# savelovme/adaptive-mcmc

Measured on AMD Instinct MI355X. Metric: chain-steps/sec (whole node) + ESS/sec, 64-dim Gaussian, higher is better.
Workload: dtype f32; 1 GPU; ARWMH.sample, d=64 correlated Gaussian, 65536 chains, per-chain adaptation (BASELINE.json configs[1]); chains_per_gpu=65536, dim=64, parallelism=1 GPU

## Files before the change

adaptive-mcmc_amd/csrc/amh_step64.hip:

```cpp
#include "amh_asss.h"
#include "amh_device.h"
#include "amh_s64_sched.h"
#include "amh_step_stage.h"

namespace amh {

#ifdef AMH_STAMPS
constexpr int kS64StampWaves = 1 << 16;
constexpr int kS64StampSlots = 8;
__device__ unsigned long long g_s64_stamps[kS64StampWaves * kS64StampSlots];
hipError_t diag_s64_stamps_copy(void* host, size_t bytes) {
  return hipMemcpyFromSymbol(host, HIP_SYMBOL(g_s64_stamps), bytes, 0, hipMemcpyDeviceToHost);
}
#define AMH_S64_PHASE_INIT unsigned long long st_ph[4] = {0, 0, 0, 0}, st_pt = 0;
#define AMH_S64_PHASE_MARK st_pt = __builtin_amdgcn_s_memrealtime();
#define AMH_S64_PHASE(k)                                             \
  {                                                                  \
    const unsigned long long t_ = __builtin_amdgcn_s_memrealtime();  \
    st_ph[k] += t_ - st_pt;                                          \
    st_pt = t_;                                                      \
  }
#else
#define AMH_S64_PHASE_INIT
#define AMH_S64_PHASE_MARK
#define AMH_S64_PHASE(k)
#endif

constexpr int kS64Waves = 16;
constexpr int kS64LoadAuxHot = 2, kS64LoadAuxCold = 2;
constexpr int kS64StoreAuxHot = 2, kS64StoreAuxMid = 0, kS64StoreAuxTail = 0;
constexpr int kS64TagShift = 60;
constexpr int64_t kS64IdxMask = ((int64_t)1 << kS64TagShift) - 1;
__device__ __forceinline__ int s64_cls(int64_t t) { return (int)(t >> kS64TagShift); }
template <class F>
__device__ __forceinline__ void s64_load_policy(int cls, F&& f) {
  using std::integral_constant;
  if constexpr (kS64LoadAuxHot == kS64LoadAuxCold) {
    f(integral_constant<int, kS64LoadAuxCold>{});
  } else {
    if (cls & (int)kS64Hot) f(integral_constant<int, kS64LoadAuxHot>{});
    else f(integral_constant<int, kS64LoadAuxCold>{});
  }
}
template <class F>
__device__ __forceinline__ void s64_store_policy(int cls, F&& f) {
  using std::integral_constant;
  if constexpr (kS64StoreAuxHot == kS64StoreAuxMid && kS64StoreAuxTail == kS64StoreAuxMid) {
    f(integral_constant<int, kS64StoreAuxMid>{});
  } else {
    if (cls & (int)kS64Hot) f(integral_constant<int, kS64StoreAuxHot>{});
    else if (cls & (int)kS64Tail) f(integral_constant<int, kS64StoreAuxTail>{});
    else f(integral_constant<int, kS64StoreAuxMid>{});
  }
}
constexpr int kS64EB = 8;
constexpr int kS64PB = 8;
static_assert(kS64EB == 8 && kS64PB == 8, "the batch readers (lds_ld4x2w / lds_ld4x4w) read two quarter-vectors per stream");
typedef uint32_t uint32x4_t_ __attribute__((ext_vector_type(4)));
constexpr int kS64P = 2080;
constexpr int kS64Z = 2080, kS64M = 2144, kS64S = 2208, kS64X = 2216;
constexpr int kS64WB = kS64X + 64;
constexpr int kS64Model = 64 * 68;
static_assert(kS64Z == 2080 && kS64S == kS64M + 64, "layout of prefetch_item<64>");
template <int WPB = kS64Waves>
constexpr size_t s64_lds_bytes() { return ((size_t)kS64Model + (size_t)WPB * kS64WB + 32) * sizeof(float); }

constexpr int s64_col(int j) { return j * 64 - j * (j - 1) / 2; }

constexpr int kS64Pieces = 9;
constexpr int s64_piece_end(int m) { return m < kS64Pieces - 1 ? 256 * (m + 1) : kS64P; }
constexpr int s64_piece_group(int m) {
  for (int g = 0; g < 16; ++g)
    if (s64_col(4 * g + 4) >= s64_piece_end(m)) return g;
  return -1;
}
constexpr int s64_piece_after(int g) {
  for (int m = 0; m < kS64Pieces; ++m)
    if (s64_piece_group(m) == g) return m;
  return -1;
}
constexpr bool s64_pieces_ok() {
  int n = 0;
  for (int g = 0; g < 16; ++g) n += s64_piece_after(g) >= 0;
  for (int m = 0; m + 1 < kS64Pieces; ++m)
    if (s64_piece_group(m) < 0 || s64_piece_group(m) >= s64_piece_group(m + 1)) return false;
  return n == kS64Pieces;
}
static_assert(256 * (kS64Pieces - 1) <= kS64P && kS64P - 256 * (kS64Pieces - 1) <= 64, "eight 1-KB pieces and a one-DMA tail");
static_assert(s64_col(64) == kS64P && s64_pieces_ok(), "every piece is finished by its own swap group, in order");
static_assert(s64_piece_group(0) == 1 && s64_piece_group(4) == 6 && s64_piece_group(7) == 14 &&
                  s64_piece_group(kS64Pieces - 1) == 15,
              "the table of DESIGN.md 3.1");

#define AMH_SWG_RD(k) "s_lshl_b64 exec, -1, %[m" #k "]\n\tds_read_b32 %[t" #k "], %[la] offset:%[o" #k "]\n\t"
#define AMH_SWG_RD_HEAD "ds_read_b128 %[dl], %[zm] offset:%[od]\n\tds_read_b128 %[in], %[zm] offset:%[oi]\n\t"
#define AMH_SWG_RD_PIECE "ds_read_b128 %[pv], %[lp] offset:%[op]\n\t"
#define AMH_SWG_RD_TAIL "s_mov_b64 exec, -1\n\ts_waitcnt lgkmcnt(0)"
template <int G, int MP>
__device__ __forceinline__ void s64_group_read(f32x4& dl4, f32x4& in4, f32x4& pv, float (&t)[4], uint32_t zm_a,
                                               uint32_t la16, uint32_t la) {
  constexpr int j = 4 * G;
  static_assert(G < 15 || MP >= 0, "the last group reads the piece that group 14 finished");
#define AMH_SWG_RD_OPS3                                                                                       \
  [zm] "v"(zm_a), [la] "v"(la), [od] "n"(16 * G), [oi] "n"(256 + 16 * G), [m0] "n"(j + 1), [m1] "n"(j + 2), \
      [m2] "n"(j + 3), [o0] "n"((s64_col(j) - j) * 4), [o1] "n"((s64_col(j + 1) - (j + 1)) * 4),             \
      [o2] "n"((s64_col(j + 2) - (j + 2)) * 4)
  if constexpr (G == 15) {
    asm volatile(AMH_SWG_RD_HEAD AMH_SWG_RD_PIECE AMH_SWG_RD(0) AMH_SWG_RD(1) AMH_SWG_RD(2) AMH_SWG_RD_TAIL
                 : [dl] "=&v"(dl4), [in] "=&v"(in4), [pv] "=&v"(pv), [t0] "=&v"(t[0]), [t1] "=&v"(t[1]),
                   [t2] "=&v"(t[2])
                 : AMH_SWG_RD_OPS3, [lp] "v"(la16), [op] "n"(1024 * MP));
  } else if constexpr (MP >= 0) {
    asm volatile(AMH_SWG_RD_HEAD AMH_SWG_RD_PIECE AMH_SWG_RD(0) AMH_SWG_RD(1) AMH_SWG_RD(2) AMH_SWG_RD(3)
                     AMH_SWG_RD_TAIL
                 : [dl] "=&v"(dl4), [in] "=&v"(in4), [pv] "=&v"(pv), [t0] "=&v"(t[0]), [t1] "=&v"(t[1]),
                   [t2] "=&v"(t[2]), [t3] "=&v"(t[3])
                 : AMH_SWG_RD_OPS3, [m3] "n"(j + 4), [o3] "n"((s64_col(j + 3) - (j + 3)) * 4), [lp] "v"(la16),
                   [op] "n"(1024 * MP));
  } else {
    asm volatile(AMH_SWG_RD_HEAD AMH_SWG_RD(0) AMH_SWG_RD(1) AMH_SWG_RD(2) AMH_SWG_RD(3) AMH_SWG_RD_TAIL
                 : [dl] "=&v"(dl4), [in] "=&v"(in4), [t0] "=&v"(t[0]), [t1] "=&v"(t[1]), [t2] "=&v"(t[2]),
                   [t3] "=&v"(t[3])
                 : AMH_SWG_RD_OPS3, [m3] "n"(j + 4), [o3] "n"((s64_col(j + 3) - (j + 3)) * 4));
  }
#undef AMH_SWG_RD_OPS3
}
#define AMH_SWG_LP                                                                      \
  "v_mul_f32 %[d0], %[u0], %[d0]\n\tv_mul_f32 %[d1], %[u1], %[d1]\n\t"                  \
  "v_mul_f32 %[d2], %[u2], %[d2]\n\tv_mul_f32 %[d3], %[u3], %[d3]\n\t"
#define AMH_SWG_WR(k) "ds_write_b32 %[la], %[d" #k "] offset:%[o" #k "]\n\t"
#define AMH_SWG_NRM(k) "v_mul_f32 %[u" #k "], %[t" #k "], %[i" #k "]\n\t"
#define AMH_SWG_SH(k) "s_lshl_b64 exec, -1, %[m" #k "]\n\t"
#define AMH_SWG_OFFS                                                                                          \
  [o0] "n"((s64_col(j) - j) * 4), [o1] "n"((s64_col(j + 1) - (j + 1)) * 4),                                   \
      [o2] "n"((s64_col(j + 2) - (j + 2)) * 4), [o3] "n"((s64_col(j + 3) - (j + 3)) * 4), [m0] "n"(j),        \
      [m1] "n"(j + 1), [m2] "n"(j + 2), [m3] "n"(j + 3)
template <int G>
__device__ __forceinline__ void s64_group_write(const float (&U)[64], uint32_t la, const f32x4& dl4) {
  constexpr int j = 4 * G;
  float d0 = dl4[0], d1 = dl4[1], d2 = dl4[2], d3 = dl4[3];
  asm volatile(AMH_SWG_LP AMH_SWG_SH(0) AMH_SWG_WR(0) AMH_SWG_SH(1) AMH_SWG_WR(1) AMH_SWG_SH(2) AMH_SWG_WR(2)
                   AMH_SWG_SH(3) AMH_SWG_WR(3) "s_mov_b64 exec, -1"
               : [d0] "+v"(d0), [d1] "+v"(d1), [d2] "+v"(d2), [d3] "+v"(d3)
               : [la] "v"(la), [u0] "v"(U[j]), [u1] "v"(U[j + 1]), [u2] "v"(U[j + 2]), [u3] "v"(U[j + 3]), AMH_SWG_OFFS
               : "memory");
}
template <int G>
__device__ __forceinline__ void s64_group_norm(float (&U)[64], const f32x4& in4, const float (&t)[4]) {
  constexpr int j = 4 * G;
  if constexpr (G < 15) {
    asm volatile(AMH_SWG_SH(1) AMH_SWG_NRM(0) AMH_SWG_SH(2) AMH_SWG_NRM(1) AMH_SWG_SH(3) AMH_SWG_NRM(2) AMH_SWG_SH(4)
                     AMH_SWG_NRM(3) "s_mov_b64 exec, -1"
                 : [u0] "+v"(U[j]), [u1] "+v"(U[j + 1]), [u2] "+v"(U[j + 2]), [u3] "+v"(U[j + 3])
                 : [t0] "v"(t[0]), [t1] "v"(t[1]), [t2] "v"(t[2]), [t3] "v"(t[3]), [i0] "v"(in4[0]), [i1] "v"(in4[1]),
                   [i2] "v"(in4[2]), [i3] "v"(in4[3]), [m1] "n"(j + 1), [m2] "n"(j + 2), [m3] "n"(j + 3),
                   [m4] "n"(j + 4));
  } else {
    asm volatile(AMH_SWG_SH(1) AMH_SWG_NRM(0) AMH_SWG_SH(2) AMH_SWG_NRM(1) AMH_SWG_SH(3) AMH_SWG_NRM(2)
                 "s_mov_b64 exec, -1"
                 : [u0] "+v"(U[j]), [u1] "+v"(U[j + 1]), [u2] "+v"(U[j + 2])
                 : [t0] "v"(t[0]), [t1] "v"(t[1]), [t2] "v"(t[2]), [i0] "v"(in4[0]), [i1] "v"(in4[1]),
                   [i2] "v"(in4[2]), [m1] "n"(j + 1), [m2] "n"(j + 2), [m3] "n"(j + 3));
  }
}
template <int O0, int O1>
__device__ __forceinline__ void lds_ld4x2w(f32x4& a, f32x4& b, uint32_t addr) {
  asm volatile("ds_read_b128 %0, %2 offset:%3\n\tds_read_b128 %1, %2 offset:%4\n\ts_waitcnt lgkmcnt(0)"
               : "=&v"(a), "=&v"(b)
               : "v"(addr), "n"(O0), "n"(O1));
}
template <int O0, int O1, int O2, int O3>
__device__ __forceinline__ void lds_ld4x4w(f32x4& a, f32x4& b, f32x4& c, f32x4& d, uint32_t addr0, uint32_t addr1) {
  asm volatile("ds_read_b128 %0, %4 offset:%6\n\tds_read_b128 %1, %4 offset:%7\n\t"
               "ds_read_b128 %2, %5 offset:%8\n\tds_read_b128 %3, %5 offset:%9\n\ts_waitcnt lgkmcnt(0)"
               : "=&v"(a), "=&v"(b), "=&v"(c), "=&v"(d)
               : "v"(addr0), "v"(addr1), "n"(O0), "n"(O1), "n"(O2), "n"(O3));
}

#define AMH_SW1_COL(k)                                                          \
  "s_lshl_b64 exec, -1, %[s" #k "]\n\tv_readlane_b32 %[t], %[w], %[l" #k "]\n\t" \
  "s_nop 1\n\tv_fma_f32 %[w], -%[t], %[u" #k "], %[w]\n\ts_nop 0\n\t"
template <int J0>
__device__ __forceinline__ void s64_sweep1x8(float& w, const float (&U)[64]) {
  uint64_t sv;
  uint32_t t;
  if constexpr (J0 + 7 <= 62) {
    asm volatile("s_mov_b64 %[sv], exec\n\t" AMH_SW1_COL(0) AMH_SW1_COL(1) AMH_SW1_COL(2) AMH_SW1_COL(3)
                 AMH_SW1_COL(4) AMH_SW1_COL(5) AMH_SW1_COL(6) AMH_SW1_COL(7) "s_mov_b64 exec, %[sv]"
                 : [w] "+v"(w), [t] "=&s"(t), [sv] "=&s"(sv)
                 : [u0] "v"(U[J0]), [u1] "v"(U[J0 + 1]), [u2] "v"(U[J0 + 2]), [u3] "v"(U[J0 + 3]),
                   [u4] "v"(U[J0 + 4]), [u5] "v"(U[J0 + 5]), [u6] "v"(U[J0 + 6]), [u7] "v"(U[J0 + 7]),
                   [s0] "n"(J0 + 1), [s1] "n"(J0 + 2), [s2] "n"(J0 + 3), [s3] "n"(J0 + 4), [s4] "n"(J0 + 5),
                   [s5] "n"(J0 + 6), [s6] "n"(J0 + 7), [s7] "n"(J0 + 8), [l0] "n"(J0), [l1] "n"(J0 + 1),
                   [l2] "n"(J0 + 2), [l3] "n"(J0 + 3), [l4] "n"(J0 + 4), [l5] "n"(J0 + 5), [l6] "n"(J0 + 6),
                   [l7] "n"(J0 + 7));
  } else {
    static_assert(J0 == 56, "sweep 1 covers columns 0 .. 62");
    asm volatile("s_mov_b64 %[sv], exec\n\t" AMH_SW1_COL(0) AMH_SW1_COL(1) AMH_SW1_COL(2) AMH_SW1_COL(3)
                 AMH_SW1_COL(4) AMH_SW1_COL(5) AMH_SW1_COL(6) "s_mov_b64 exec, %[sv]"
                 : [w] "+v"(w), [t] "=&s"(t), [sv] "=&s"(sv)
                 : [u0] "v"(U[J0]), [u1] "v"(U[J0 + 1]), [u2] "v"(U[J0 + 2]), [u3] "v"(U[J0 + 3]),
                   [u4] "v"(U[J0 + 4]), [u5] "v"(U[J0 + 5]), [u6] "v"(U[J0 + 6]), [s0] "n"(J0 + 1),
                   [s1] "n"(J0 + 2), [s2] "n"(J0 + 3), [s3] "n"(J0 + 4), [s4] "n"(J0 + 5), [s5] "n"(J0 + 6),
                   [s6] "n"(J0 + 7), [l0] "n"(J0), [l1] "n"(J0 + 1), [l2] "n"(J0 + 2), [l3] "n"(J0 + 3),
                   [l4] "n"(J0 + 4), [l5] "n"(J0 + 5), [l6] "n"(J0 + 6));
  }
}
#undef AMH_SW1_COL
__device__ __forceinline__ void s64_sweep1_all(float& w, const float (&U)[64]) {
  static_for<8>([&](auto B) {
    s64_sweep1x8<8 * B>(w, U);
    __builtin_amdgcn_sched_barrier(0);
  });
}

template <int Q>
__device__ __forceinline__ void s64_wr4_quarter(uint32_t a, float v0, float v1, float v2, float v3) {
  uint64_t sv;
  asm volatile("s_mov_b64 %0, exec\n\ts_bfm_b64 exec, 16, %6\n\tds_write_b32 %1, %2\n\t"
               "ds_write_b32 %1, %3 offset:64\n\tds_write_b32 %1, %4 offset:128\n\t"
               "ds_write_b32 %1, %5 offset:192\n\ts_mov_b64 exec, %0"
               : "=&s"(sv) : "v"(a), "v"(v0), "v"(v1), "v"(v2), "v"(v3), "n"(16 * Q) : "memory");
}
__device__ __forceinline__ void s64_wr(uint32_t a, float v) {
  asm volatile("ds_write_b32 %0, %1" : : "v"(a), "v"(v) : "memory");
}
template <int OFF>
__device__ __forceinline__ void s64_wr_off(uint32_t a, float v) {
  asm volatile("ds_write_b32 %0, %1 offset:%2" : : "v"(a), "v"(v), "n"(OFF) : "memory");
}
__device__ __forceinline__ void s64_wait() { asm volatile("s_waitcnt lgkmcnt(0)" ::: "memory"); }
template <class T>
__device__ __forceinline__ void s64_tie(T& a) { asm volatile("s_waitcnt lgkmcnt(0)" : "+v"(a)); }
template <class T>
__device__ __forceinline__ void s64_tie(T& a, T& b) { asm volatile("s_waitcnt lgkmcnt(0)" : "+v"(a), "+v"(b)); }

template <int J>
__device__ __forceinline__ float s64_keep_at(float old, float v) {
  float out;
  unsigned long long m;
  asm("s_lshl_b64 %1, 1, %4\n\tv_cndmask_b32_e64 %0, %2, %3, %1" : "=v"(out), "=&s"(m) : "v"(old), "v"(v), "n"(J));
  return out;
}

template <bool WAIT = false>
__device__ __forceinline__ float s64_matvec(const float (&U)[64], float h, uint32_t x_a, uint32_t r) {
  s64_wr(x_a + r * 4u, h);
  float a4[4] = {0.0f, 0.0f, 0.0f, 0.0f};
  static_for<64 / kS64EB>([&](auto B) {
    constexpr int b = B;
    f32x4 e[kS64EB / 4];
    lds_ld4x2w<16 * (2 * b), 16 * (2 * b + 1)>(e[0], e[1], x_a);
    static_for<kS64EB>([&](auto K) {
      constexpr int j = kS64EB * b + K;
      a4[j & 3] = fmaf(U[j], e[(int)K / 4][(int)K % 4], a4[j & 3]);
    });
    __builtin_amdgcn_sched_barrier(0);
  });
  if constexpr (WAIT) s64_wait();
  return (a4[0] + a4[1]) + (a4[2] + a4[3]);
}

__device__ __forceinline__ float s64_gauss_pot(float diff, uint32_t x_a, uint32_t prow, uint32_t r, float c0) {
  s64_wr(x_a + r * 4u, diff);
  f32x2v y01 = {0.0f, 0.0f}, y23 = {0.0f, 0.0f};
  static_for<64 / kS64PB>([&](auto B) {
    constexpr int b = B;
    constexpr int NQ = kS64PB / 4;
    f32x4 pv[NQ], dv[NQ];
    lds_ld4x4w<16 * (2 * b), 16 * (2 * b + 1), 16 * (2 * b), 16 * (2 * b + 1)>(pv[0], pv[1], dv[0], dv[1], prow, x_a);
    static_for<2 * NQ>([&](auto K2) {
      const f32x4 q = pv[(int)K2 / 2];
      const f32x4 dq = dv[(int)K2 / 2];
      const f32x2v pp = (K2 % 2 == 0) ? f32x2v{q[0], q[1]} : f32x2v{q[2], q[3]};
      const f32x2v bp = (K2 % 2 == 0) ? f32x2v{dq[0], dq[1]} : f32x2v{dq[2], dq[3]};
      if constexpr (K2 % 2 == 0) {
        y01 = __builtin_elementwise_fma(pp, bp, y01);
      } else {
        y23 = __builtin_elementwise_fma(pp, bp, y23);
      }
    });
    __builtin_amdgcn_sched_barrier(0);
  });
  const float y = (y01[0] + y01[1]) + (y23[0] + y23[1]);
  const float S = Grp<64>::sum(diff * y);
  return (0.5f * S) + c0;
}

struct S64Coef {
  bool revert;
  float c, q;
};
__device__ __forceinline__ S64Coef s64_rank_one_coef(float ws, float Dg, float one, float gamma, int r) {
  using Gp = Grp<64>;
  const float gw2 = gamma * (ws * ws);
  const float tsc = gw2 / Dg;
  const float b = 1.0f + Gp::excl_scan(tsc, r);
  const float g2 = (b * Dg) + gw2;
  const float dn = g2 / b;
  const float c = (gamma * ws) / g2;
  const float q = sqrtf(dn);
  const float dnew = fmaf(c, 0.0f, one) * q;
  return {Gp::any(amh_isnan(dnew)), c, q};
}
__device__ __forceinline__ float s64_sweep2(float (&U)[64], float delta, float ws, float c, float ac, float bc,
                                            uint32_t x_a, uint32_t xq_a) {
  float s4[4] = {0.0f, 0.0f, 0.0f, 0.0f};
  float w = delta;
  static_for<16>([&](auto G4) {
    constexpr int g = G4;
    if constexpr (g % 4 == 0) s64_wr4_quarter<g / 4>(xq_a, ws, c, ac, bc);
    constexpr int gq = g % 4;
    f32x4 cw, cc, ca, cb;
    lds_ld4x4w<16 * gq, 64 + 16 * gq, 128 + 16 * gq, 192 + 16 * gq>(cw, cc, ca, cb, x_a, x_a);
    static_for<4>([&](auto Q) {
      constexpr int j = 4 * g + Q;
      const float uo = U[j];
      w = fmaf(-cw[(int)Q], uo, w);
      const float un = fmaf(cc[(int)Q], w, uo);
      const float tt = fmaf(uo, ca[(int)Q], cb[(int)Q] * w);
      s4[j & 3] = fmaf(tt, tt, s4[j & 3]);
      U[j] = un;
    });
    column_fence<g, 2>();
  });
  const float sacc = (s4[0] + s4[1]) + (s4[2] + s4[3]);
  return Grp<64>::sum(sacc);
}

__device__ __forceinline__ void asss_transition64(const StepParams& p, float (&U)[64], float& dl, float& x, float& mu,
                                                  float& pe, float& asc, bool& updated, int32_t it, uint32_t k0,
                                                  uint32_t k1, int r, const GaussianM<64>::Ctx& mctx, uint32_t x_a,
                                                  uint32_t xq_a, uint32_t prow) {
  using Gp = Grp<64>;
  constexpr int d = 64;
  const float sd = sqrtf((float)d);
  const float epsd = p.eps * sd;
  const float fd = (float)d;
  const uint32_t ur = (uint32_t)r;
  const amh_u32x4 o = amh_philox4x32_10((uint32_t)r, (uint32_t)it, 0u, AMH_TAG_ASSS, k0, k1);
  float v = amh_normal_from_bits(o.v[0]);
  float vd = amh_normal_from_bits(Gp::template bcast_u<0>(o.v[1]));
  const float ut = amh_unif01_from_bits(Gp::template bcast_u<0>(o.v[2]));
  const float th0 = 6.28318548f * amh_unif01_from_bits(Gp::template bcast_u<0>(o.v[3]));

  const float e = dl * sd;
  const float Dr = (dl + p.eps) * sd;
  const float invD = 1.0f / Dr;
  float b = x - mu;
  float y = 0.0f;
  static_for<d>([&](auto J) {
    constexpr int j = J;
    const float yl = b * invD;
    y = s64_keep_at<j>(y, yl);
    const float gj = Gp::template bcast<j>(yl * e);
    b = fmaf(-U[j], gj, b);
    column_fence<j>();
  });

  const float ns = Gp::sum(y * y);
  const float den = ns + 1.0f;
  const float zr = (2.0f * y) / den;
  const float zd = (ns - 1.0f) / den;

  const float dot = Gp::sum(v * zr) + (vd * zd);
  v = fmaf(-dot, zr, v);
  vd = fmaf(-dot, zd, vd);
  const float nv = sqrtf(Gp::sum(v * v) + (vd * vd));
  const bool degen = !(nv > 0.0f);
  v = degen ? 0.0f : v / nv;
  vd = degen ? 0.0f : vd / nv;

  const float Sz = s64_matvec<true>(U, e * zr, x_a, ur) + epsd * zr;
  const float Sv = s64_matvec<true>(U, e * v, x_a, ur) + epsd * v;

  auto x_at = [&](float c, float s, float& om) -> float {
    const float zdt = (zd * c) + (vd * s);
    om = 1.0f - zdt;
    return (((Sz * c) + (Sv * s)) / om) + mu;
  };
  auto pot = [&](float xv) -> float {
    const float u = s64_gauss_pot(xv - mctx.mr, x_a, prow, ur, mctx.c0);
    s64_wait();
    return u;
  };

  float om0;
  const float x0 = x_at(1.0f, 0.0f, om0);
  const float U0 = pot(x0);
  const float tpe = (U0 + fd * amh_logf(om0)) - amh_logf(ut);

  float th = th0, thmin = th0 - 6.28318548f, thmax = th0;
  int32_t iter = 0;
  float xt, ux;
  bool cont;
  {
    float s, c, om;
    amh_sincosf(th, &s, &c);
    xt = x_at(c, s, om);
    ux = pot(xt);
    float pt = ux + fd * amh_logf(om);
    if (amh_isnan(pt)) pt = INFINITY;
    cont = !degen && ((pt > tpe) || (om < p.eps));
  }
  while (cont) {
    const float thmin_n = (th < 0.0f) ? th : thmin;
    const float thmax_n = (th >= 0.0f) ? th : thmax;
    const amh_u32x4 ok = amh_philox4x32_10((uint32_t)iter, (uint32_t)it, 1u, AMH_TAG_ASSS, k0, k1);
    const float th_n = thmin_n + (thmax_n - thmin_n) * amh_unif01_from_bits(ok.v[0]);
    float s, c, om;
    amh_sincosf(th_n, &s, &c);
    const float xn = x_at(c, s, om);
    const float un = pot(xn);
    float pt = un + fd * amh_logf(om);
    if (amh_isnan(pt)) pt = INFINITY;
    thmin = thmin_n;
    thmax = thmax_n;
    th = th_n;
    xt = xn;
    ux = un;
    iter += 1;
    cont = (iter < kAsssMaxIter) && ((pt > tpe) || (om < p.eps));
  }
  const bool capped = degen || iter >= kAsssMaxIter;
  const float xnew = capped ? x0 : xt;
  float pen = capped ? U0 : ux;
  if (amh_isnan(pen)) pen = INFINITY;

  const int32_t itr = it + 1;
  const int32_t n = (it < p.W) ? itr : itr - p.W;
  const float gamma = lookup_gamma<64>(p, n);
  const float delta = xnew - mu;
  const float mun = mu + gamma * delta;
  const float dmu = mun - mu;
  const float locd = sqrtf(Gp::sum(dmu * dmu));

  const float sq = sqrtf(1.0f - gamma);
  const float ajj = sq * dl;
  const float Dg = ajj * ajj;
  const float one = (amh_isfinite(ajj) && ajj != 0.0f) ? 1.0f : __int_as_float(0x7FC00000);
  float ws = delta;
  s64_sweep1_all(ws, U);
  const S64Coef k = s64_rank_one_coef(ws, Dg, one, gamma, r);
  float sdiff = 0.0f;
  if (!k.revert) {
    sdiff = sqrtf(s64_sweep2(U, delta, ws, k.c, k.q - dl, k.c * k.q, x_a, xq_a));
    dl = k.q;
    updated = true;
  }
  asc = locd + sdiff;
  x = xnew;
  pe = pen;
  mu = mun;
}

__device__ __forceinline__ void arwmh_transition64(const StepParams& p, float (&U)[64], float& dl, float& z, float& mu,
                                                   float& pe, float& macc, float& lam, float& asc, bool& updated,
                                                   int32_t& nacc, int32_t it, uint32_t k0, uint32_t k1, int r,
                                                   const GaussianM<64>::Ctx& mctx, uint32_t x_a, uint32_t xq_a,
                                                   uint32_t prow) {
  using Gp = Grp<64>;
  float xi, u;
  step_noise_w64(r, (uint32_t)it, k0, k1, xi, u);

  const float el = amh_expf(lam);
  const float eta = dl * xi;
  const float acc = s64_matvec(U, eta, x_a, (uint32_t)r);
  const float zp = z + fmaf(el, acc, p.eps * xi);

  float pep = s64_gauss_pot(zp - mctx.mr, x_a, prow, (uint32_t)r, mctx.c0);
  if (amh_isnan(pep)) pep = INFINITY;

  const float ex = amh_expf(pe - pep);
  const float alpha = (ex > 1.0f) ? 1.0f : ex;
  const bool accept = u < alpha;
  const float zn = accept ? zp : z;
  const float pen = accept ? pep : pe;
  nacc += accept ? 1 : 0;

  const int32_t itr = it + 1;
  const int32_t n = (it < p.W) ? itr : itr - p.W;
  const float gamma = lookup_gamma<64>(p, n);
  const float maccn = macc + (alpha - macc) / (float)n;

  const float delta = zn - mu;
  const float mun = mu + gamma * delta;
  const float lamn = lam + gamma * (alpha - p.target);
  const float e1 = amh_expf(lamn);

  const float sq = sqrtf(1.0f - gamma);
  const float ajj = sq * dl;
  const float Dg = ajj * ajj;
  const float one = (amh_isfinite(ajj) && ajj != 0.0f) ? 1.0f : __int_as_float(0x7FC00000);

  float ws = delta;
  s64_sweep1_all(ws, U);

  const S64Coef k = s64_rank_one_coef(ws, Dg, one, gamma, r);
  if (!k.revert) {
    const float ac = (k.q * e1) - (dl * el);
    const float bc = (k.c * k.q) * e1;
    asc = sqrtf(s64_sweep2(U, delta, ws, k.c, ac, bc, x_a, xq_a));
    dl = k.q;
    updated = true;
  } else {
    const float ac = (dl * e1) - (dl * el);
    float s4[4] = {0.0f, 0.0f, 0.0f, 0.0f};
    static_for<64>([&](auto J) {
      const float tt = U[J] * Gp::template bcast<J>(ac);
      s4[J & 3] = fmaf(tt, tt, s4[J & 3]);
      column_fence<J>();
    });
    const float sacc = (s4[0] + s4[1]) + (s4[2] + s4[3]);
    asc = sqrtf(Gp::sum(sacc));
  }

  z = zn;
  pe = pen;
  macc = maccn;
  mu = mun;
  lam = lamn;
}

template <int WPB, bool kASSS = false>
__global__ __launch_bounds__(WPB * 64) void arwmh_step64_kernel(StepParams p) {
  const StepParams& p_outer = p;
  constexpr int D = 64;
  constexpr uint32_t P = kS64P;
  static_assert(WPB >= 1 && (WPB * 64) % 64 == 0, "d = 64 step kernel: every wave of the block is full");
  using Gp = Grp<64>;
  using M = GaussianM<64>;
  extern __shared__ float lds[];
  M::stage(lds, p.model, D);
  float* tick = lds + kS64Model + WPB * kS64WB;
  const int64_t blk_lo = p.C * (int64_t)blockIdx.x / gridDim.x;
  const int64_t blk_hi = p.C * ((int64_t)blockIdx.x + 1) / gridDim.x;
  const uint32_t tk_step = p.descending ? ~0u : 1u;
  if (threadIdx.x == 0) {
    const S64Sched sch = s64_sched((uint32_t)(blk_hi - blk_lo), p.descending, p.chained);
    tick[0] = __uint_as_float(sch.first);
    tick[4] = __uint_as_float(sch.hot_lo);
    tick[5] = __uint_as_float(sch.hot_n);
    tick[6] = __uint_as_float(sch.tail_lo);
    tick[7] = __uint_as_float(sch.tail_n);
  }
  __syncthreads();
  const auto mctx = M::prepare(p.model, D, lane_id());
#ifdef AMH_STAMPS
  const unsigned long long st_start = __builtin_amdgcn_s_memrealtime();
  int st_items = 0;
#endif
  AMH_S64_PHASE_INIT

  const int64_t C = p.C;
  const int wave_in_block = __builtin_amdgcn_readfirstlane((int)(threadIdx.x / 64));
  float* wb = lds + kS64Model + wave_in_block * kS64WB;
  const uint32_t wb_a = lds_addr(wb);
  const uint32_t x_a = wb_a + kS64X * 4;
  const uint32_t zm_a = wb_a + kS64Z * 4;
  const uint32_t xq_a = x_a + (uint32_t)(lane_id() & 15) * 4u;
  const uint32_t prow = lds_addr(lds) + (uint32_t)lane_id() * (uint32_t)(M::ld(D) * 4);

  float U[D];
  static_for<D>([&](auto J) { U[J] = set_one_at<64, J>(0.0f, lane_id()); });
  float dl = 0.0f, z = 0.0f, mu = 0.0f, pe = 0.0f, macc = 0.0f, lam = 0.0f, asc = 0.0f;
  int32_t it = 0, nacc = 0, acc0 = 0;
  uint32_t k0 = 0, k1 = 0;
  int64_t prev = -1;
  bool prev_upd = false;

  const int64_t kEnd = blk_hi;
  const uint32_t tk_addr = lds_addr(tick);
  auto ticket = [&]() -> int64_t {
    uint32_t v = 0;
    if (lane_id() == 0) {
      uint32x4_t_ b;
      asm volatile("ds_add_rtn_u32 %0, %2, %3\n\tds_read_b128 %1, %2 offset:16\n\ts_waitcnt lgkmcnt(0)"
                   : "=&v"(v), "=&v"(b) : "v"(tk_addr), "v"(tk_step) : "memory");
      const uint32_t cls = s64_class(v, b[0], b[1], b[2], b[3]);
      v = (v < 0x3FFFFFFFu ? v : 0x3FFFFFFFu) | (cls << 30);
    }
    const uint32_t w = (uint32_t)__builtin_amdgcn_readfirstlane((int)v);
    return (blk_lo + (int64_t)(w & 0x3FFFFFFFu)) | ((int64_t)(w >> 30) << kS64TagShift);
  };
  auto ix = [](int64_t t) -> int64_t { return t & kS64IdxMask; };
  auto prefetch = [&](int64_t t, int ln) {
    s64_load_policy(s64_cls(t), [&](auto AUX) { prefetch_item<64, false, decltype(AUX)::value>(p, ix(t), D, wb, ln); });
  };

  auto store_small = [&](int64_t c, int r) {
    const StepParams& p = reload_kernarg(p_outer);
    p.out.z[c * D + r] = z;
    p.out.loc[c * D + r] = mu;
    if (r == 0) {
      p.out.i[c] = it;
      p.out.potential_energy[c] = pe;
      if constexpr (!kASSS) {
        p.out.mean_accept_prob[c] = macc;
        p.out.log_step_size[c] = lam;
      }
      p.out.as_change[c] = asc;
      p.out.rng_key[2 * c] = k0;
      p.out.rng_key[2 * c + 1] = k1;
      if (!kASSS && p.accept_count != nullptr) p.accept_count[c] = acc0 + nacc;
    }
  };
  auto copy_verbatim = [&](int64_t c, int r) {
    const uint32_t vrow = (uint32_t)r * 4u;
    const Buf Lout(uniform_ptr(p.out.scale + c * P), P * 4u);
    const Buf Lin(uniform_ptr(p.in.scale + c * P), P * 4u);
    static_for<4>([&](auto B) {
      static_for<16>([&](auto K) {
        constexpr int j = 16 * B + K;
        U[j] = Lin.ld(off_from<64, j>(vrow, kOOB, r), (uint32_t)(s64_col(j) - j) * 4u);
      });
      static_for<16>([&](auto K) {
        constexpr int j = 16 * B + K;
        Lout.st(U[j], off_from<64, j>(vrow, kOOB, r), (uint32_t)(s64_col(j) - j) * 4u);
      });
      __builtin_amdgcn_sched_barrier(0);
    });
    __builtin_amdgcn_s_waitcnt(0);
    static_for<D>([&](auto J) { U[J] = set_one_at<64, J>(0.0f, r); });
  };
  auto flush_aux = [&](int64_t c, auto AUX) {
    const Buf Lout(uniform_ptr(p.out.scale + c * P), P * 4u);
    const uint32_t la = wb_a + (uint32_t)lane_id() * 16u;
    static_for<3>([&](auto G) {
      f32x4 v[3];
      static_for<3>([&](auto Q) { v[(int)Q] = lds_ld4<1024 * (3 * G + Q)>(la); });
      asm volatile("s_waitcnt lgkmcnt(0)" : "+v"(v[0]), "+v"(v[1]), "+v"(v[2]));
      static_for<3>([&](auto Q) {
        __builtin_amdgcn_raw_buffer_store_b128(__builtin_bit_cast(uint32x4_t_, v[(int)Q]), Lout.rs,
                                               (int)(1024u * (3 * G + Q) + 16u * (uint32_t)lane_id()), 0,
                                               (int)AUX);
      });
    });
  };
  auto flush_factor = [&](int64_t t) {
    s64_store_policy(s64_cls(t), [&](auto AUX) { flush_aux(ix(t), AUX); });
  };

  int64_t item = ticket();
  int64_t nxt = ix(item) < kEnd ? ticket() : kEnd;
  if (ix(item) < kEnd) prefetch(item, lane_id());
  for (; ix(item) < kEnd;) {
    int lane = lane_id();
    asm volatile("" : "+v"(lane));
    const int r = lane;
    const uint32_t la = wb_a + (uint32_t)r * 4u;

    AMH_S64_PHASE_MARK
    __builtin_amdgcn_s_waitcnt(0x0F70);
    AMH_S64_PHASE(0)
    __builtin_amdgcn_s_setprio(3);
    if (prev >= 0) store_small(ix(prev), r);
    const bool wr = prev >= 0 && prev_upd;
    if (prev >= 0 && !prev_upd) copy_verbatim(ix(prev), r);

    float lnew = lds_ld1<0>(wb_a + (uint32_t)s64_col(r) * 4u);
    s64_tie(lnew);
    const float inv = (amh_isfinite(lnew) && lnew != 0.0f) ? 1.0f / lnew : 0.0f;
    {
      float zz = lds_ld1<kS64Z * 4>(la), mm = lds_ld1<kS64M * 4>(la);
      const uint32_t sa = wb_a + kS64S * 4;
      float s0 = lds_ld1<0>(sa), s1 = lds_ld1<4>(sa), s2 = lds_ld1<8>(sa), s3 = lds_ld1<12>(sa);
      float s4v = lds_ld1<16>(sa), s5 = lds_ld1<20>(sa), s6 = lds_ld1<24>(sa);
      asm volatile("s_waitcnt lgkmcnt(0)" : "+v"(zz), "+v"(mm), "+v"(s0), "+v"(s1), "+v"(s2), "+v"(s3), "+v"(s4v),
                   "+v"(s5), "+v"(s6));
      z = zz;
      mu = mm;
      it = __builtin_amdgcn_readfirstlane(__float_as_int(s0));
      pe = s1;
      macc = s2;
      lam = s3;
      asc = s4v;
      k0 = (uint32_t)__builtin_amdgcn_readfirstlane(__float_as_int(s5));
      k1 = (uint32_t)__builtin_amdgcn_readfirstlane(__float_as_int(s6));
      s64_wr(zm_a + (uint32_t)r * 4u, dl);
      s64_wr_off<256>(zm_a + (uint32_t)r * 4u, inv);
      dl = lnew;
      acc0 = (!kASSS && p.accept_count != nullptr && r == 0) ? p.accept_count[ix(item)] : 0;
    }

    const bool have_nxt = ix(nxt) < kEnd;
    const Buf Lnx(uniform_ptr(p.in.scale + ix(nxt) * P), P * 4u);
    auto piece_in = [&](auto M) {
      constexpr int m = M;
      if (!have_nxt) return;
      uint32_t base = wb_a;
      asm volatile("" : "+s"(base));
      lds_void* dst = (lds_void*)(uintptr_t)(base + 1024u * m);
      s64_load_policy(s64_cls(nxt), [&](auto AUX) {
        if constexpr (m < kS64Pieces - 1) {
          __builtin_amdgcn_raw_ptr_buffer_load_lds(Lnx.rs, dst, 16, (int)(16u * lane), 1024 * m, 0, (int)AUX);
        } else {
          if (256 * m + lane < kS64P)
            __builtin_amdgcn_raw_ptr_buffer_load_lds(Lnx.rs, dst, 4, (int)(4u * lane), 1024 * m, 0, (int)AUX);
        }
      });
    };
    const Buf Lout(uniform_ptr(p.out.scale + ix(wr ? prev : item) * P), P * 4u);
    const int cls = s64_cls(prev);
    const uint32_t la16 = wb_a + (uint32_t)lane * 16u;
    auto piece_out = [&](auto M, const f32x4& v) {
      constexpr int m = M;
      s64_store_policy(cls, [&](auto AUX) {
        __builtin_amdgcn_raw_buffer_store_b128(__builtin_bit_cast(uint32x4_t_, v), Lout.rs,
                                               (int)(16u * (uint32_t)lane), 1024 * m, (int)AUX);
      });
    };
    static_for<16>([&](auto G4) {
      constexpr int g = G4;
      constexpr int mp = g > 0 ? s64_piece_after(g - 1) : -1;
      f32x4 dl4, in4, pv;
      float t[4];
      s64_group_read<g, mp>(dl4, in4, pv, t, zm_a, la16, la);
      if (wr) {
        if constexpr (mp >= 0) {
          piece_out(std::integral_constant<int, mp>{}, pv);
          piece_in(std::integral_constant<int, mp>{});
          if constexpr (mp == 0) {
            AMH_S64_PHASE(1)
          }
        }
        s64_group_write<g>(U, la, dl4);
      }
      s64_group_norm<g>(U, in4, t);
    });
    if (wr) {
      constexpr int mp = s64_piece_after(15);
      static_assert(mp == kS64Pieces - 1, "the last group finishes the tail");
      f32x4 pv = lds_ld4<1024 * mp>(la16);
      s64_tie(pv);
      piece_out(std::integral_constant<int, mp>{}, pv);
      piece_in(std::integral_constant<int, mp>{});
    } else {
      AMH_S64_PHASE(1)
      s64_wait();
      static_for<kS64Pieces>([&](auto M) { piece_in(M); });
    }

    s64_wait();
    int64_t nxt2 = kEnd;
    if (have_nxt) {
      prefetch_item_small<64, false>(p, ix(nxt), D, wb, lane);
      nxt2 = ticket();
    }
    __builtin_amdgcn_s_setprio(0);
    AMH_S64_PHASE(2)

    nacc = 0;
    bool updated = false;
    for (int32_t t = 0; t < p.n_steps; ++t) {
      if constexpr (kASSS) {
        asss_transition64(p, U, dl, z, mu, pe, asc, updated, it, k0, k1, r, mctx, x_a, xq_a, prow);
      } else {
        arwmh_transition64(p, U, dl, z, mu, pe, macc, lam, asc, updated, nacc, it, k0, k1, r, mctx, x_a, xq_a, prow);
      }
      it += 1;
      if (p.col_z != nullptr || p.col_pe != nullptr) {
        if ((t + 1) % p.thinning == 0) {
          const int64_t kk = t / p.thinning;
          if (p.col_z != nullptr) p.col_z[(kk * C + ix(item)) * D + r] = z;
          if (p.col_pe != nullptr && r == 0) p.col_pe[kk * C + ix(item)] = pe;
        }
      }
    }
    prev = item;
    prev_upd = Gp::any(updated);
    item = nxt;
    nxt = nxt2;
    AMH_S64_PHASE(3)
#ifdef AMH_STAMPS
    ++st_items;
#endif
  }
  if (prev >= 0) {
    int lane = lane_id();
    asm volatile("" : "+v"(lane));
    const uint32_t la = wb_a + (uint32_t)lane * 4u;
    store_small(ix(prev), lane);
    if (prev_upd) {
      s64_wr(x_a + (uint32_t)lane * 4u, dl);
      static_for<16>([&](auto G4) {
        constexpr int g = G4;
        f32x4 dl4 = lds_ld4<16 * g>(x_a);
        s64_tie(dl4);
        s64_group_write<g>(U, la, dl4);
      });
      flush_factor(prev);
    } else {
      copy_verbatim(ix(prev), lane);
    }
  }
  __builtin_amdgcn_s_waitcnt(0);
#ifdef AMH_STAMPS
  {
    const unsigned long long st_end = __builtin_amdgcn_s_memrealtime();
    const int64_t w = (int64_t)blockIdx.x * WPB + wave_in_block;
    if (w < kS64StampWaves && lane_id() == 0) {
      unsigned long long* row = g_s64_stamps + w * kS64StampSlots;
      row[0] = st_start;
      row[1] = st_end;
      row[2] = (unsigned long long)st_items;
      row[3] = (unsigned long long)blockIdx.x;
      for (int k_ = 0; k_ < 4; ++k_) row[4 + k_] = st_ph[k_];
    }
  }
#endif
}

template <int WPB, bool kASSS = false>
hipError_t launch_step64(const StepParams& p, hipStream_t s) {
  constexpr size_t shm = s64_lds_bytes<WPB>();
  static_assert(shm <= 163840, "d = 64 step kernel: LDS budget");
  auto kern = arwmh_step64_kernel<WPB, kASSS>;
  int per_cu = 0;
  hipError_t e = hipOccupancyMaxActiveBlocksPerMultiprocessor(&per_cu, kern, WPB * 64, shm);
  if (e != hipSuccess) return e;
  const int cus = cu_count();
  if (per_cu < 1) per_cu = 1;
  const int64_t need = (p.C + WPB - 1) / WPB;
  int64_t blocks = (int64_t)cus * per_cu;
  if (blocks > need) blocks = need;
  if (blocks < 1) blocks = 1;
  hipLaunchKernelGGL(kern, dim3((unsigned)blocks), dim3(WPB * 64), shm, s, p);
  return hipGetLastError();
}

hipError_t run_step64(const StepParams& p, hipStream_t s) { return launch_step64<kS64Waves>(p, s); }
constexpr int kAsss64Waves = 16;
hipError_t run_asss_step64(const StepParams& p, hipStream_t s) {
  return launch_step64<kAsss64Waves, true>(p, s);
}

}
```

Before: 319.1 million chain-steps/s.

## Broadcast matvec and potential operands via readlane when each item runs one step

```diff
diff --git a/adaptive-mcmc_amd/csrc/amh_step64.hip b/adaptive-mcmc_amd/csrc/amh_step64.hip
--- a/adaptive-mcmc_amd/csrc/amh_step64.hip
+++ b/adaptive-mcmc_amd/csrc/amh_step64.hip
@@ -7,12 +7,15 @@
 
 #ifdef AMH_STAMPS
 constexpr int kS64StampWaves = 1 << 16;
-constexpr int kS64StampSlots = 8;
+constexpr int kS64StampSlots = 16;
+constexpr int kS64SubPhases = 6;
 __device__ unsigned long long g_s64_stamps[kS64StampWaves * kS64StampSlots];
 hipError_t diag_s64_stamps_copy(void* host, size_t bytes) {
   return hipMemcpyFromSymbol(host, HIP_SYMBOL(g_s64_stamps), bytes, 0, hipMemcpyDeviceToHost);
 }
-#define AMH_S64_PHASE_INIT unsigned long long st_ph[4] = {0, 0, 0, 0}, st_pt = 0;
+#define AMH_S64_PHASE_INIT                                  \
+  unsigned long long st_ph[4] = {0, 0, 0, 0}, st_pt = 0; \
+  S64Sub st_sub = {{0, 0, 0, 0, 0, 0}, 0};
 #define AMH_S64_PHASE_MARK st_pt = __builtin_amdgcn_s_memrealtime();
 #define AMH_S64_PHASE(k)                                             \
   {                                                                  \
@@ -20,10 +23,26 @@
     st_ph[k] += t_ - st_pt;                                          \
     st_pt = t_;                                                      \
   }
+struct S64Sub {
+  unsigned long long ph[kS64SubPhases], pt;
+};
+#define AMH_S64_SUB_PARAM , S64Sub& st_sub
+#define AMH_S64_SUB_ARG , st_sub
+#define AMH_S64_SUB_MARK st_sub.pt = __builtin_amdgcn_s_memrealtime();
+#define AMH_S64_SUB(k)                                               \
+  {                                                                  \
+    const unsigned long long t_ = __builtin_amdgcn_s_memrealtime();  \
+    st_sub.ph[k] += t_ - st_sub.pt;                                  \
+    st_sub.pt = t_;                                                  \
+  }
 #else
 #define AMH_S64_PHASE_INIT
 #define AMH_S64_PHASE_MARK
 #define AMH_S64_PHASE(k)
+#define AMH_S64_SUB_PARAM
+#define AMH_S64_SUB_ARG
+#define AMH_S64_SUB_MARK
+#define AMH_S64_SUB(k)
 #endif
 
 constexpr int kS64Waves = 16;
@@ -55,7 +74,9 @@
 }
 constexpr int kS64EB = 8;
 constexpr int kS64PB = 8;
+constexpr int kS64PG = 16;
 static_assert(kS64EB == 8 && kS64PB == 8, "the batch readers (lds_ld4x2w / lds_ld4x4w) read two quarter-vectors per stream");
+static_assert(kS64PG == 16, "s64_gauss_pot_sg waits for four quarter-rows; s64_lanes takes 8 or 16");
 typedef uint32_t uint32x4_t_ __attribute__((ext_vector_type(4)));
 constexpr int kS64P = 2080;
 constexpr int kS64Z = 2080, kS64M = 2144, kS64S = 2208, kS64X = 2216;
@@ -92,18 +113,19 @@
                   s64_piece_group(kS64Pieces - 1) == 15,
               "the table of DESIGN.md 3.1");
 
-#define AMH_SWG_RD(k) "s_lshl_b64 exec, -1, %[m" #k "]\n\tds_read_b32 %[t" #k "], %[la] offset:%[o" #k "]\n\t"
+#define AMH_SWG_RD(k) "ds_read_b32 %[t" #k "], %[la] offset:%[o" #k "]\n\t"
 #define AMH_SWG_RD_HEAD "ds_read_b128 %[dl], %[zm] offset:%[od]\n\tds_read_b128 %[in], %[zm] offset:%[oi]\n\t"
 #define AMH_SWG_RD_PIECE "ds_read_b128 %[pv], %[lp] offset:%[op]\n\t"
-#define AMH_SWG_RD_TAIL "s_mov_b64 exec, -1\n\ts_waitcnt lgkmcnt(0)"
+#define AMH_SWG_RD_TAIL "s_waitcnt lgkmcnt(0)"
 template <int G, int MP>
 __device__ __forceinline__ void s64_group_read(f32x4& dl4, f32x4& in4, f32x4& pv, float (&t)[4], uint32_t zm_a,
                                                uint32_t la16, uint32_t la) {
   constexpr int j = 4 * G;
   static_assert(G < 15 || MP >= 0, "the last group reads the piece that group 14 finished");
-#define AMH_SWG_RD_OPS3                                                                                       \
-  [zm] "v"(zm_a), [la] "v"(la), [od] "n"(16 * G), [oi] "n"(256 + 16 * G), [m0] "n"(j + 1), [m1] "n"(j + 2), \
-      [m2] "n"(j + 3), [o0] "n"((s64_col(j) - j) * 4), [o1] "n"((s64_col(j + 1) - (j + 1)) * 4),             \
+  static_assert(s64_col(j) >= j && s64_col(j + 3) - (j + 3) + 63 < kS64P, "unmasked column reads stay inside the factor");
+#define AMH_SWG_RD_OPS3                                                                          \
+  [zm] "v"(zm_a), [la] "v"(la), [od] "n"(16 * G), [oi] "n"(256 + 16 * G),                       \
+      [o0] "n"((s64_col(j) - j) * 4), [o1] "n"((s64_col(j + 1) - (j + 1)) * 4),                 \
       [o2] "n"((s64_col(j + 2) - (j + 2)) * 4)
   if constexpr (G == 15) {
     asm volatile(AMH_SWG_RD_HEAD AMH_SWG_RD_PIECE AMH_SWG_RD(0) AMH_SWG_RD(1) AMH_SWG_RD(2) AMH_SWG_RD_TAIL
@@ -115,13 +137,12 @@
                      AMH_SWG_RD_TAIL
                  : [dl] "=&v"(dl4), [in] "=&v"(in4), [pv] "=&v"(pv), [t0] "=&v"(t[0]), [t1] "=&v"(t[1]),
                    [t2] "=&v"(t[2]), [t3] "=&v"(t[3])
-                 : AMH_SWG_RD_OPS3, [m3] "n"(j + 4), [o3] "n"((s64_col(j + 3) - (j + 3)) * 4), [lp] "v"(la16),
-                   [op] "n"(1024 * MP));
+                 : AMH_SWG_RD_OPS3, [o3] "n"((s64_col(j + 3) - (j + 3)) * 4), [lp] "v"(la16), [op] "n"(1024 * MP));
   } else {
     asm volatile(AMH_SWG_RD_HEAD AMH_SWG_RD(0) AMH_SWG_RD(1) AMH_SWG_RD(2) AMH_SWG_RD(3) AMH_SWG_RD_TAIL
                  : [dl] "=&v"(dl4), [in] "=&v"(in4), [t0] "=&v"(t[0]), [t1] "=&v"(t[1]), [t2] "=&v"(t[2]),
                    [t3] "=&v"(t[3])
-                 : AMH_SWG_RD_OPS3, [m3] "n"(j + 4), [o3] "n"((s64_col(j + 3) - (j + 3)) * 4));
+                 : AMH_SWG_RD_OPS3, [o3] "n"((s64_col(j + 3) - (j + 3)) * 4));
   }
 #undef AMH_SWG_RD_OPS3
 }
@@ -243,6 +264,60 @@
   return out;
 }
 
+template <int J0, int N>
+__device__ __forceinline__ void s64_lanes(float v, float (&s)[N]) {
+  static_assert(N == 8 || N == 16, "batches of 8 or 16 lanes");
+  static_for<N>([&](auto K) { s[(int)K] = __int_as_float(__builtin_amdgcn_readlane(__float_as_int(v), J0 + K)); });
+  if constexpr (N == 8) {
+    asm volatile("" : "+s"(s[0]), "+s"(s[1]), "+s"(s[2]), "+s"(s[3]), "+s"(s[4]), "+s"(s[5]), "+s"(s[6]), "+s"(s[7]));
+  } else {
+    asm volatile("" : "+s"(s[0]), "+s"(s[1]), "+s"(s[2]), "+s"(s[3]), "+s"(s[4]), "+s"(s[5]), "+s"(s[6]), "+s"(s[7]),
+                 "+s"(s[8]), "+s"(s[9]), "+s"(s[10]), "+s"(s[11]), "+s"(s[12]), "+s"(s[13]), "+s"(s[14]), "+s"(s[15]));
+  }
+}
+
+__device__ __forceinline__ float s64_matvec_sg(const float (&U)[64], float h) {
+  float a4[4] = {0.0f, 0.0f, 0.0f, 0.0f};
+  static_for<64 / kS64EB>([&](auto B) {
+    constexpr int b = B;
+    float e[kS64EB];
+    s64_lanes<kS64EB * b>(h, e);
+    static_for<kS64EB>([&](auto K) {
+      constexpr int j = kS64EB * b + K;
+      a4[j & 3] = fmaf(U[j], e[(int)K], a4[j & 3]);
+    });
+    __builtin_amdgcn_sched_barrier(0);
+  });
+  return (a4[0] + a4[1]) + (a4[2] + a4[3]);
+}
+
+__device__ __forceinline__ float s64_gauss_pot_sg(float diff, uint32_t prow, float c0) {
+  f32x2v y01 = {0.0f, 0.0f}, y23 = {0.0f, 0.0f};
+  static_for<64 / kS64PG>([&](auto B) {
+    constexpr int b = B;
+    constexpr int NQ = kS64PG / 4;
+    f32x4 pv[NQ];
+    static_for<NQ>([&](auto Q) { pv[(int)Q] = lds_ld4<16 * (NQ * b + Q)>(prow); });
+    float dv[kS64PG];
+    s64_lanes<kS64PG * b>(diff, dv);
+    asm volatile("s_waitcnt lgkmcnt(0)" : "+v"(pv[0]), "+v"(pv[1]), "+v"(pv[2]), "+v"(pv[3]));
+    static_for<2 * NQ>([&](auto K2) {
+      const f32x4 q = pv[(int)K2 / 2];
+      const f32x2v pp = (K2 % 2 == 0) ? f32x2v{q[0], q[1]} : f32x2v{q[2], q[3]};
+      const f32x2v bp = {dv[2 * (int)K2], dv[2 * (int)K2 + 1]};
+      if constexpr (K2 % 2 == 0) {
+        y01 = __builtin_elementwise_fma(pp, bp, y01);
+      } else {
+        y23 = __builtin_elementwise_fma(pp, bp, y23);
+      }
+    });
+    __builtin_amdgcn_sched_barrier(0);
+  });
+  const float y = (y01[0] + y01[1]) + (y23[0] + y23[1]);
+  const float S = Grp<64>::sum(diff * y);
+  return (0.5f * S) + c0;
+}
+
 template <bool WAIT = false>
 __device__ __forceinline__ float s64_matvec(const float (&U)[64], float h, uint32_t x_a, uint32_t r) {
   s64_wr(x_a + r * 4u, h);
@@ -458,18 +533,23 @@
                                                    float& pe, float& macc, float& lam, float& asc, bool& updated,
                                                    int32_t& nacc, int32_t it, uint32_t k0, uint32_t k1, int r,
                                                    const GaussianM<64>::Ctx& mctx, uint32_t x_a, uint32_t xq_a,
-                                                   uint32_t prow) {
+                                                   uint32_t prow, bool sg AMH_S64_SUB_PARAM) {
   using Gp = Grp<64>;
+  AMH_S64_SUB_MARK
   float xi, u;
   step_noise_w64(r, (uint32_t)it, k0, k1, xi, u);
 
+  AMH_S64_SUB(0)
   const float el = amh_expf(lam);
   const float eta = dl * xi;
-  const float acc = s64_matvec(U, eta, x_a, (uint32_t)r);
+  const float acc = sg ? s64_matvec_sg(U, eta) : s64_matvec(U, eta, x_a, (uint32_t)r);
   const float zp = z + fmaf(el, acc, p.eps * xi);
 
-  float pep = s64_gauss_pot(zp - mctx.mr, x_a, prow, (uint32_t)r, mctx.c0);
+  AMH_S64_SUB(1)
+  float pep = sg ? s64_gauss_pot_sg(zp - mctx.mr, prow, mctx.c0)
+                 : s64_gauss_pot(zp - mctx.mr, x_a, prow, (uint32_t)r, mctx.c0);
   if (amh_isnan(pep)) pep = INFINITY;
+  AMH_S64_SUB(2)
 
   const float ex = amh_expf(pe - pep);
   const float alpha = (ex > 1.0f) ? 1.0f : ex;
@@ -493,10 +573,12 @@
   const float Dg = ajj * ajj;
   const float one = (amh_isfinite(ajj) && ajj != 0.0f) ? 1.0f : __int_as_float(0x7FC00000);
 
+  AMH_S64_SUB(3)
   float ws = delta;
   s64_sweep1_all(ws, U);
 
   const S64Coef k = s64_rank_one_coef(ws, Dg, one, gamma, r);
+  AMH_S64_SUB(4)
   if (!k.revert) {
     const float ac = (k.q * e1) - (dl * el);
     const float bc = (k.c * k.q) * e1;
@@ -515,6 +597,7 @@
     asc = sqrtf(Gp::sum(sacc));
   }
 
+  AMH_S64_SUB(5)
   z = zn;
   pe = pen;
   macc = maccn;
@@ -752,11 +835,13 @@
 
     nacc = 0;
     bool updated = false;
+    const bool sg = p.n_steps == 1;
     for (int32_t t = 0; t < p.n_steps; ++t) {
       if constexpr (kASSS) {
         asss_transition64(p, U, dl, z, mu, pe, asc, updated, it, k0, k1, r, mctx, x_a, xq_a, prow);
       } else {
-        arwmh_transition64(p, U, dl, z, mu, pe, macc, lam, asc, updated, nacc, it, k0, k1, r, mctx, x_a, xq_a, prow);
+        arwmh_transition64(p, U, dl, z, mu, pe, macc, lam, asc, updated, nacc, it, k0, k1, r, mctx, x_a, xq_a, prow,
+                           sg AMH_S64_SUB_ARG);
       }
       it += 1;
       if (p.col_z != nullptr || p.col_pe != nullptr) {
@@ -806,6 +891,7 @@
       row[2] = (unsigned long long)st_items;
       row[3] = (unsigned long long)blockIdx.x;
       for (int k_ = 0; k_ < 4; ++k_) row[4 + k_] = st_ph[k_];
+      for (int k_ = 0; k_ < kS64SubPhases; ++k_) row[8 + k_] = st_sub.ph[k_];
     }
   }
 #endif
```

After: 323.0 million chain-steps/s, median of 6. 1.2% higher.
